# huangzhibo/Hadoop-BAM

Measured on AMD Instinct MI355X. Metric: uncompressed BAM decode GB/s + records/sec per GPU and 8-GPU node, higher is better.
Workload: dtype u8; 1 GPU; C2: synthetic 10M x 150bp paired-end coordinate-sorted BAM; records_per_gpu=10000000, uncompressed_bytes=3401886473, split_bytes_rank0=1410310329, parallelism=FileVirtualSplit per rank x1 (BAMSplitGuesser)

## Files before the change

hadoop-bam_amd/csrc/hbam_abi.cpp:

```cpp
#include "../../include/hbam.h"

#include <hip/hip_runtime.h>

#include <algorithm>
#include <cstdio>
#include <cstdlib>
#include <cstring>
#include <map>
#include <memory>
#include <mutex>
#include <string>
#include <vector>

#include "hbam_deflate_api.h"
#include "hbam_mem.h"
#include "hbam_host.h"
#include "hbam_launch.h"

using hadoop_bam::BAMInputFormat;
using hadoop_bam::BamFile;
using hadoop_bam::BAMRecordReader;
using hadoop_bam::Carry;
using hadoop_bam::FileSplit;
using hadoop_bam::FileVirtualSplit;
// ... 428 lines not shown
  }
  return ctx->cursor.reader_position(i, pos, &ctx->err);
}

int hbam_pipeline_counters(hbam_ctx* ctx, uint64_t out[5]) {
  if (!ctx || !ctx->f) return HBAM_E_STATE;
  hbam::Pipeline& p = ctx->f->pipe();
  out[0] = p.link_fallbacks();
  out[1] = p.link_rewalks();
  out[2] = p.record_fallbacks();
  out[3] = p.inflate_launches();
  out[4] = p.records_after_stop();
  return HBAM_OK;
}

int hbam_inflate_token_count(hbam_ctx* ctx, uint64_t* tokens) {
  *tokens = 0;
  if (!ctx || !ctx->f) return HBAM_E_STATE;
  return ctx->f->pipe().inflate_tokens(tokens) == 0 ? HBAM_OK : HBAM_E_DEVICE;
}

int hbam_inflate_path_counts(hbam_ctx* ctx, uint64_t out[3]) {
  out[0] = out[1] = out[2] = 0;
  if (!ctx || !ctx->f) return HBAM_E_STATE;
  return ctx->f->pipe().inflate_path_counts(out) == 0 ? HBAM_OK : HBAM_E_DEVICE;
}

int hbam_inflate_narrow_counts(hbam_ctx* ctx, uint64_t out[3]) {
  out[0] = out[1] = out[2] = 0;
  if (!ctx || !ctx->f) return HBAM_E_STATE;
// ... 442 lines not shown
  return rc;
}

int hbam_gpu_set_window(hbam_gpu* g, uint64_t window_bytes) {
  g->window = window_bytes ? window_bytes : hadoop_bam::kDefaultWindowBytes;
  if (g->f) g->f->set_window_bytes(g->window);
  return HBAM_OK;
}

int hbam_gpu_set_stringency(hbam_gpu* g, int32_t stringency) {
  if (stringency < HBAM_STRICT || stringency > HBAM_SILENT) {
    g->err = "unknown validation stringency";
    return HBAM_E_ARG;
  }
  g->stringency = stringency;
  return HBAM_OK;
}

int hbam_gpu_run(hbam_gpu* g, int32_t flags, hbam_gpu_stats* st) {
  memset(st, 0, sizeof *st);
  if (!g->f) {
    g->err = "hbam_gpu_run needs a loaded file";
    return HBAM_E_STATE;
  }
  return decode_device(*g->f, g->f->first_record_voff(), ~0ull, flags, st, &g->span, &g->err);
}

int hbam_gpu_index(hbam_gpu* g, int32_t granularity, uint8_t** buf, uint64_t* len, float* ms) {
  *buf = nullptr;
  *len = 0;
// ... 263 lines not shown
```

hadoop-bam_amd/csrc/hbam_kernels.hip:

```cpp
#include <hip/hip_runtime.h>
#include <hipcub/hipcub.hpp>
#include <stddef.h>
#include <stdint.h>

#include "hbam_device.h"
#include "hbam_launch.h"

namespace hbam {

__device__ __forceinline__ uint32_t rfl(uint32_t v) { return __builtin_amdgcn_readfirstlane(v); }
__device__ __forceinline__ uint32_t lane_id() { return __lane_id(); }

__device__ __forceinline__ uint32_t ldu32(const uint8_t* base, uint64_t off) {
  const uint32_t* p = reinterpret_cast<const uint32_t*>(base + (off & ~3ull));
  uint32_t lo = p[0], hi = p[1];
  return __builtin_amdgcn_alignbyte(hi, lo, (uint32_t)(off & 3));
}
__device__ __forceinline__ uint64_t ldu64(const uint8_t* base, uint64_t off) {
  return (uint64_t)ldu32(base, off) | ((uint64_t)ldu32(base, off + 4) << 32);
}

struct __attribute__((aligned(4))) U32x4 { uint32_t x, y, z, w; };
struct __attribute__((aligned(4))) U32x2 { uint32_t x, y; };
struct RecHead {
// ... 88 lines not shown
          s_cand[j] = base + p;
        } else {
          const uint32_t i = atomicAdd(count, 1u);
          if (i < cap) cand[i] = base + p;
        }
      }
    }
    }
  }
  __syncthreads();
  const uint32_t nw = min(s_n, kWgCand);
  if (threadIdx.x == 0) s_base = nw ? atomicAdd(count, nw) : 0u;
  __syncthreads();
  for (uint32_t t = threadIdx.x; t < nw; t += blockDim.x)
    if (s_base + t < cap) cand[s_base + t] = s_cand[t];
}

__global__ void k_bgzf_verify(const uint8_t* __restrict__ file, uint64_t lo, uint64_t hi,
                              const uint64_t* __restrict__ cand, uint32_t n,
                              BlockInfo* __restrict__ blocks, uint32_t* __restrict__ flags, uint32_t partial) {
  uint32_t i = blockIdx.x * blockDim.x + threadIdx.x;
  if (i >= n) return;
  uint64_t c = cand[i];
  if (i == 0 && c != lo) atomicOr(&flags[0], 1u);
  uint32_t total = (ldu32(file, c + 16) & 0xffffu) + 1;
  uint64_t next = c + total;
  uint64_t expect = (i + 1 < n) ? cand[i + 1] : hi;
  if (partial && i + 1 == n && next > hi && total >= 26) {
    flags[2] = 1u;
    return;
// ... 3529 lines not shown
  uint64_t g = (n + bs - 1) / bs;
  if (g < 1) g = 1;
  if (g > cap) g = cap;
  return (unsigned)g;
}

hipError_t launch_bgzf_scan(const uint8_t* file, uint64_t buf_base, uint64_t lo, uint64_t hi, uint64_t* cand,
                            uint32_t cap, uint32_t* count, hipStream_t s) {
  (void)buf_base;
  const uint64_t a = lo & ~15ull;
  const uint64_t nc = (hi - a + 15) / 16;
  hipLaunchKernelGGL(k_bgzf_scan, dim3(grid_for((nc + 3) / 4, 256, HBAM_SCAN_GRID)), dim3(256), 0, s, file + a, hi - a, a, lo,
                     cand, cap, count);
  return hipGetLastError();
}
hipError_t launch_bgzf_verify(const uint8_t* file, uint64_t lo, uint64_t hi, const uint64_t* cand, uint32_t n,
                              BlockInfo* blocks, uint32_t* flags, uint32_t partial, hipStream_t s) {
  if (n == 0) return hipSuccess;
  hipLaunchKernelGGL(k_bgzf_verify, dim3((n + 255) / 256), dim3(256), 0, s, file, lo, hi, cand, n, blocks, flags,
                     partial);
  return hipGetLastError();
}
hipError_t launch_bgzf_walk(const uint8_t* file, uint64_t lo, uint64_t hi, BlockInfo* blocks, uint32_t cap,
                            uint32_t* out, uint32_t partial, hipStream_t s) {
  hipLaunchKernelGGL(k_bgzf_walk, dim3(1), dim3(64), 0, s, file, lo, hi, blocks, cap, out, partial);
  return hipGetLastError();
}
hipError_t launch_block_ustart(BlockInfo* blocks, uint32_t n, uint64_t* tmp_isize, uint64_t* tmp_ustart,
                               void* scan_tmp, size_t* scan_bytes, uint64_t base, hipStream_t s) {
  if (scan_tmp == nullptr) {
// ... 295 lines not shown
```

hadoop-bam_amd/csrc/hbam_launch.h:

```cpp
#pragma once
#include <hip/hip_runtime.h>
#include <stdint.h>

#include "hbam_device.h"

namespace hbam {

struct ChainArgs {
  const uint8_t* u;
  const BlockInfo* blocks;
  uint64_t e_inf, e_true, p0, q_end;
  const uint64_t* dead;
  uint32_t ndead;
  int32_t n_ref;
  uint32_t k0, k1;
  int validate;
  const int32_t* ref_len;
  uint64_t *g, *x, *entry, *summary, *base;
  uint64_t* x2;
  void* scan_tmp;
  size_t scan_bytes;
  uint32_t* cnt;
  int32_t* err;
  unsigned long long* need;
// ... 18 lines not shown
  kStageSerialLink = 1,
  kStageCount = 2,
  kStageEmit = 3,
  kStageWalk = 5,
  kStageLinkCheck = 6,
  kStageRewalk = 7,
  kStageRewalkAll = 8,
};

hipError_t launch_bgzf_scan(const uint8_t* file, uint64_t buf_base, uint64_t lo, uint64_t hi, uint64_t* cand,
                            uint32_t cap, uint32_t* count, hipStream_t s);
hipError_t launch_bgzf_verify(const uint8_t* file, uint64_t lo, uint64_t hi, const uint64_t* cand, uint32_t n,
                              BlockInfo* blocks, uint32_t* flags, uint32_t partial, hipStream_t s);
hipError_t launch_bgzf_walk(const uint8_t* file, uint64_t lo, uint64_t hi, BlockInfo* blocks, uint32_t cap,
                            uint32_t* out, uint32_t partial, hipStream_t s);
hipError_t launch_block_ustart(BlockInfo* blocks, uint32_t n, uint64_t* tmp_isize, uint64_t* tmp_ustart,
                               void* scan_tmp, size_t* scan_bytes, uint64_t base, hipStream_t s);
hipError_t sort_u64(void* tmp, size_t* tmp_bytes, uint64_t* keys_in, uint64_t* keys_out, uint32_t n,
                    hipStream_t s);
hipError_t scan_u32_to_u64(void* tmp, size_t* tmp_bytes, const uint32_t* in, uint64_t* out, uint32_t n,
                           hipStream_t s);
hipError_t launch_huff_tables(const uint8_t* file, const BlockInfo* blocks, uint32_t b0, uint32_t nb,
                              uint8_t* tables, HuffTableInfo* tinfo, const HuffOut* hout, uint32_t round,
                              hipStream_t s);
hipError_t launch_inflate_huff_prebuilt(const uint8_t* file, const BlockInfo* blocks, uint32_t b0, uint32_t nb,
                                        uint64_t chunk_ustart, uint32_t* tokens, HuffOut* hout,
                                        const uint8_t* tables, const HuffTableInfo* tinfo, uint32_t round,
                                        uint32_t defer, uint32_t* flist, uint32_t* pstats, hipStream_t s);
hipError_t huff_lean_occupancy(int* workgroups_per_cu);
hipError_t huff_narrow_occupancy(int* workgroups_per_cu, uint32_t* stage_cap_bytes);
// ... 45 lines not shown
```

hadoop-bam_amd/csrc/hbam_pipeline.cpp:

```cpp
#include "hbam_pipeline.h"

#include <thread>

#include <algorithm>
#include <chrono>
#include <cstdio>
#include <cstdlib>
#include <cstring>

#include "hbam_launch.h"

namespace hbam {

namespace {
constexpr uint32_t kStreamInflateBlocks = 8192;
#ifndef HBAM_INFLATE_CHUNK
#define HBAM_INFLATE_CHUNK 65536
#endif
constexpr uint32_t kInflateChunkBlocks = HBAM_INFLATE_CHUNK;
constexpr int kMaxChainIters = 64;
constexpr int kMaxLinkFix = 4;
constexpr int kMaxFreeStarts = 64;
constexpr uint64_t kOpenEnd = 1ull << 62;
}
// ... 18 lines not shown
      create_stream(&stream_stage_, StreamLevel::kLow) != hipSuccess)
    err_ = "hipStreamCreate failed";
  streams_.s[0] = stream_;
  streams_.s[1] = stream_b_;
  streams_.s[2] = stream_t_;
  streams_.s[3] = stream_copy_;
  streams_.n = 4;
  stage_owner_.s[0] = stream_stage_;
  stage_owner_.s[1] = stream_;
  stage_owner_.n = 2;
  stage_.owner = &stage_owner_;
  own(own_file_, own_spare_, dblocks_, ref_len_, du_, tokens_[0], tokens_[1], hout_, tables_[0], tables_[1],
      tinfo_[0], tinfo_[1], flist_[0], flist_[1], pstats_, g_, x_, x2_, entry_, base_arr_, summary_, dead_, cand_, sorted_, isz_, ust_, cnt_, flags_,
      errv_, need_, rec_pos_, rec_voff_, rcand_, force_, wcnt_, counters_, list_, scan_tmp_, cols_, long_rec_,
      long_n_, wbuf_, woffs_, wbad_, scalars_, fuse_, sort_word_, sort_word2_, sort_slen_, sort_doff_, sort_len_,
      sort_iota_, sort_perm_, sort_tmp_);
  for (auto& e : ev_) (void)hipEventCreate(&e);
  for (auto& e : sync_ev_) (void)hipEventCreateWithFlags(&e, hipEventDisableTiming);
  for (auto& e : tab_ev_) (void)hipEventCreateWithFlags(&e, hipEventDisableTiming);
  for (auto& e : hdone_ev_) (void)hipEventCreateWithFlags(&e, hipEventDisableTiming);
}

Pipeline::~Pipeline() {
  if (stage_thr_.joinable()) stage_thr_.join();
  (void)hipSetDevice(device_);
  (void)streams_.sync();
  (void)stage_owner_.sync();
  streams_.n = 0;
  stage_owner_.n = 0;
  if (rb_buf_) pinned_free(rb_buf_, rb_cap_);
  for (auto& e : ev_) (void)hipEventDestroy(e);
// ... 289 lines not shown
int Pipeline::set_ref_lengths(const std::vector<int32_t>& lens) {
  HIPCHK(ref_len_.reserve(lens.size() + 1));
  if (!lens.empty())
    HIPCHK(hipMemcpyAsync(ref_len_.p, lens.data(), lens.size() * 4, hipMemcpyHostToDevice, stream_));
  HIPCHK(rb_sync(stream_));
  n_ref_len_ = (uint32_t)lens.size();
  return kOk;
}

int Pipeline::locate_range(uint64_t lo, uint64_t hi, bool partial, bool free_start, uint32_t nprev, uint64_t ubase,
                           hipStream_t s, uint32_t* nnew, uint64_t* tail) {
  *nnew = 0;
  *tail = hi;
  const uint8_t* fbase = dfile_ - base_;
  const uint64_t len = hi - lo;
  const uint32_t cap = (uint32_t)std::min<uint64_t>(len / 1024 + 4096, 0x7fffffffu);
  const uint32_t walk_cap = (uint32_t)std::min<uint64_t>(len / 26 + 16, 0x7fffffffu);
  HIPCHK(cand_.reserve(cap));
  HIPCHK(flags_.reserve(5));
  HIPCHK(hipMemsetD32Async(reinterpret_cast<hipDeviceptr_t>(flags_.p), 0, 5, s));
  HIPCHK(hipMemsetD32Async(reinterpret_cast<hipDeviceptr_t>(flags_.p + 2), -1, 1, s));
  HIPCHK(launch_bgzf_scan(fbase, base_, lo, hi, cand_.p, cap, flags_.p, s));
  uint32_t count = 0;
  HIPCHK(rb(&count, flags_.p, 4, s));
  HIPCHK(rb_sync(s));
  bool serial = count > cap || (count == 0 && len > 0);
  if (free_start && count == 0) return kOk;
  uint32_t n = serial ? 0 : count;
  auto queue_table = [&](uint32_t nt) -> int {
    HIPCHK(dblocks_.grow(nprev + nt + 1));
    HIPCHK(isz_.reserve(nt + 1));
    HIPCHK(ust_.reserve(nt + 1));
    size_t sb = 0;
    HIPCHK(launch_block_ustart(dblocks_.p + nprev, nt, isz_.p, ust_.p, nullptr, &sb, ubase, s));
    HIPCHK(scan_tmp_.reserve(sb + 16));
    HIPCHK(launch_block_ustart(dblocks_.p + nprev, nt, isz_.p, ust_.p, scan_tmp_.p, &sb, ubase, s));
    HIPCHK(hblocks_.resize(nprev + nt));
    if (nt) HIPCHK(launch_readback(hblocks_.data() + nprev, dblocks_.p + nprev, nt * sizeof(BlockInfo), s));
    return kOk;
  };
  std::vector<uint64_t> starts;
  if (!serial && n > 0) {
    HIPCHK(dblocks_.grow(nprev + n + 1));
    HIPCHK(sorted_.reserve(n));
    size_t tmp_bytes = 0;
    HIPCHK(sort_u64(nullptr, &tmp_bytes, cand_.p, sorted_.p, n, s));
    HIPCHK(scan_tmp_.reserve(tmp_bytes + 16));
    HIPCHK(sort_u64(scan_tmp_.p, &tmp_bytes, cand_.p, sorted_.p, n, s));
    if (free_start) {
      starts.resize(std::min<uint32_t>(n, kMaxFreeStarts));
      HIPCHK(rb(starts.data(), sorted_.p, starts.size() * 8, s));
      HIPCHK(rb_sync(s));
      lo = starts[0];
    }
    HIPCHK(launch_bgzf_verify(fbase, lo, hi, sorted_.p, n, dblocks_.p + nprev, flags_.p + 1, partial ? 1u : 0u, s));
    uint32_t fl[4];
    uint64_t last = 0;
    HIPCHK(rb(fl, flags_.p + 1, 16, s));
    HIPCHK(rb(&last, sorted_.p + n - 1, 8, s));
    if (int rc = queue_table(n)) return rc;
    HIPCHK(rb_sync(s));
    if (!fl[0] && empty_blocks_ != kEmptyUnknown) empty_blocks_ += fl[3];
    if (fl[0]) serial = true;
    else if (fl[1] != 0xffffffffu) return fail(kErrFormat, "BGZF block with ISIZE > 65536 (unsupported on device)");
    else if (fl[2]) {
      n -= 1;
      *tail = last;
    }
    if (!serial) {
      HIPCHK(hblocks_.resize(nprev + n));
      *nnew = n;
      return kOk;
    }
  }
  if (serial) {
    empty_blocks_ = kEmptyUnknown;
    uint32_t out[4];
// ... 893 lines not shown
```

hadoop-bam_amd/csrc/hbam_pipeline.h:

```cpp
#pragma once
#include "hbam_feed.h"
#include "hbam_mem.h"
#include <hip/hip_runtime.h>
#include <stdint.h>

#include <algorithm>
#include <cstring>
#include <string>
#include <thread>
#include <vector>

#include "hbam_device.h"

namespace hbam {

template <typename T>
struct DevBuf {
  T* p = nullptr;
  size_t n = 0;
  const StreamSet* owner = nullptr;
  DevBuf() = default;
  explicit DevBuf(const StreamSet* o) : owner(o) {}
  DevBuf(const DevBuf&) = delete;
  DevBuf& operator=(const DevBuf&) = delete;
// ... 99 lines not shown
  uint64_t first_voff = 0, last_voff = 0;
  Columns col{};
  const uint8_t* data = nullptr;
};

struct StageTimes {
  float locate = 0, inflate = 0, huff = 0, lz77 = 0, chain = 0, decode = 0;
  float tables = 0;
};

enum class StreamLevel { kNormal, kHigh, kLow };
hipError_t create_stream(hipStream_t* s, StreamLevel level);

enum Stringency : int { kStrict = 0, kLenient = 1, kSilent = 2 };

class Pipeline {
 public:
  explicit Pipeline(int device);
  ~Pipeline();
  Pipeline(const Pipeline&) = delete;
  Pipeline& operator=(const Pipeline&) = delete;

  int device() const { return device_; }
  hipStream_t stream() const { return stream_; }
  const StreamSet& streams() const { return streams_; }
  const std::string& error() const { return err_; }

  hipError_t rb(void* dst, const void* src, size_t bytes, hipStream_t s);
  hipError_t rb_sync(hipStream_t s);
  int copy_from_host(uint8_t* dst, const HostSource& src, uint64_t off, uint64_t len);
// ... 40 lines not shown
  int64_t pos_of_voff(uint64_t voff) const;
  uint64_t voff_of(uint64_t pos) const;
  uint64_t q_end_of(uint64_t vend) const;
  uint32_t block_containing(uint64_t pos) const;

  void set_n_ref(int32_t n) { n_ref_ = n; }
  int32_t n_ref() const { return n_ref_; }
  void set_stringency(int s) { stringency_ = s; }
  int set_ref_lengths(const std::vector<int32_t>& lens);

  uint64_t link_fallbacks() const { return link_fallbacks_; }
  uint64_t link_rewalks() const { return link_rewalks_; }
  uint64_t record_fallbacks() const { return record_fallbacks_; }
  uint64_t records_after_stop() const { return records_after_stop_; }
  uint64_t inflate_launches() const { return inflate_launches_; }
  int inflate_tokens(uint64_t* n);
  int inflate_path_counts(uint64_t out[3]);
  int inflate_narrow_counts(uint64_t out[3]);
  int chain_counters(uint64_t out[4]);
  StageTimes times;
  bool timing = false;

 private:
  int fail(int code, const std::string& msg);
  int locate_range(uint64_t lo, uint64_t hi, bool partial, bool free_start, uint32_t nprev, uint64_t ubase,
                   hipStream_t s, uint32_t* nnew, uint64_t* tail);
  int finish_blocks();
  hipError_t queue_inflate_check(uint32_t b0, uint32_t b1);
  int inflate_verdict(uint32_t b0, uint32_t b1);
  uint32_t infl_first_ = 0xffffffffu;
// ... 38 lines not shown
  uint32_t ndead_ = 0;
  static constexpr uint32_t kEmptyUnknown = 0xffffffffu;
  uint32_t empty_blocks_ = kEmptyUnknown;
  int32_t n_ref_ = 0;
  int stringency_ = kStrict;
  DevBuf<int32_t> ref_len_;
  uint32_t n_ref_len_ = 0;
  uint64_t link_fallbacks_ = 0;
  uint64_t link_rewalks_ = 0;
  uint64_t link_rounds_ = 0;
  uint64_t record_fallbacks_ = 0;
  uint64_t records_after_stop_ = 0;
  uint32_t after_stop_flag_ = 0;
  bool after_stop_pending_ = false;
  uint64_t inflate_launches_ = 0;

  DevBuf<uint8_t> du_;
  std::vector<uint8_t> inflated_;
  DevBuf<uint32_t> tokens_[2];
  DevBuf<HuffOut> hout_;
  DevBuf<uint8_t> tables_[2];
  hipStream_t stream_b_ = nullptr;
  hipStream_t stream_t_ = nullptr;
  hipEvent_t tab_ev_[2];
  hipEvent_t hdone_ev_[2];
  hipEvent_t sync_ev_[4];
  DevBuf<HuffTableInfo> tinfo_[2];
  DevBuf<uint32_t> flist_[2];
  DevBuf<uint32_t> pstats_;

  DevBuf<uint64_t> g_, x_, x2_, entry_, base_arr_, summary_, dead_;
  DevBuf<uint64_t> cand_, sorted_, isz_, ust_;
  DevBuf<uint32_t> cnt_, flags_;
  DevBuf<int32_t> errv_;
  DevBuf<unsigned long long> need_;
  DevBuf<uint64_t> rec_pos_, rec_voff_;
  DevBuf<uint64_t> rcand_, force_;
  DevBuf<uint32_t> wcnt_, counters_;
  DevBuf<uint16_t> list_;
  DevBuf<uint32_t> fuse_;
  DevBuf<uint8_t> scan_tmp_;
  DevBuf<uint8_t> cols_;
  uint64_t cols_cap_ = 0;
  DevBuf<uint64_t> long_rec_;
  DevBuf<uint32_t> long_n_;
  DevBuf<uint8_t> wbuf_;
  DevBuf<uint64_t> woffs_;
  DevBuf<unsigned long long> wbad_;
// ... 20 lines not shown
```

hadoop-bam_amd/hbam/__init__.py:

```python
import ctypes as C
import os
import re

import numpy as np

_PKG = os.path.dirname(os.path.dirname(os.path.abspath(__file__)))
LIB_PATH = os.environ.get("HBAM_LIB") or os.path.join(_PKG, "lib", "libhbam.so")
HEADER_PATH = os.path.join(os.path.dirname(_PKG), "include", "hbam.h")

if not os.path.exists(LIB_PATH):
    raise ImportError(f"{LIB_PATH} is not built: run `make -C hadoop-bam_amd` (libhbam has no CPU fallback)")

_L = C.CDLL(LIB_PATH)

OK, E_FORMAT, E_TRUNC, E_ARG, E_IO, E_DEVICE, E_STATE, E_NOMEM = range(8)
ERROR_NAMES = {1: "SAMFormatException", 2: "FileTruncatedException", 3: "IllegalArgumentException",
               4: "IOException", 5: "DeviceError", 6: "IllegalStateException", 7: "OutOfMemoryError"}

u64, i64, i32, u32, P = C.c_uint64, C.c_int64, C.c_int32, C.c_uint32, C.c_void_p


STRICT, LENIENT, SILENT = 0, 1, 2


# ... 51 lines not shown
_sig("hbam_open_bgzf", C.c_int, [P, u64, C.POINTER(Opts), C.POINTER(P)])
READ_FN = C.CFUNCTYPE(C.c_int64, C.c_void_p, C.c_uint64, C.c_void_p, C.c_uint64)
_sig("hbam_open_reader", C.c_int, [u64, READ_FN, P, C.POINTER(Opts), C.POINTER(P)])
_sig("hbam_close", None, [P])
_sig("hbam_last_error", C.c_char_p, [P])
_sig("hbam_free", None, [P])
_sig("hbam_header", C.c_int, [P, C.POINTER(HeaderInfo)])
_sig("hbam_ref", C.c_int, [P, i32, C.POINTER(C.c_char_p), C.POINTER(i32)])
_sig("hbam_decode_span", C.c_int, [P, u64, u64, u64, C.POINTER(Batch)])
_sig("hbam_decode_span_device", C.c_int, [P, u64, u64, i32, C.POINTER(GpuStats)])
_sig("hbam_reader_position", C.c_int, [P, u64, C.POINTER(u64)])
_sig("hbam_query_intervals", C.c_int, [P, P, u64, P, u64])
_sig("hbam_query_unmapped", C.c_int, [P, u64])
_sig("hbam_query_next", C.c_int, [P, u64, C.POINTER(Batch)])
_sig("hbam_pipeline_counters", C.c_int, [P, C.POINTER(u64)])
_sig("hbam_inflate_token_count", C.c_int, [P, C.POINTER(u64)])
_sig("hbam_inflate_path_counts", C.c_int, [P, C.POINTER(u64)])
_sig("hbam_inflate_narrow_counts", C.c_int, [P, C.POINTER(u64)])
_sig("hbam_chain_counters", C.c_int, [P, C.POINTER(u64)])
_sig("hbam_file_stats", C.c_int, [P, C.POINTER(u64), C.POINTER(u64)])
_sig("hbam_bytes_read", C.c_int, [P, C.POINTER(u64)])
_sig("hbam_prefetch", C.c_int, [P, u64, u64])
_sig("hbam_splitting_index_for_records", C.c_int, [C.POINTER(Opts), P, u64, i32, u64, C.POINTER(P), C.POINTER(u64)])
_sig("hbam_build_splitting_index", C.c_int, [P, i32, C.POINTER(P), C.POINTER(u64)])
_sig("hbam_build_bai", C.c_int, [P, i32, C.POINTER(P), C.POINTER(u64)])
_sig("hbam_splitting_entries", C.c_int, [P, u64, u64, i32, u64, C.POINTER(P), C.POINTER(u64), C.POINTER(u64)])
_sig("hbam_guess_record_starts", C.c_int, [P, P, P, u64, P])
_sig("hbam_guess_record_starts_hdr", C.c_int, [P, i32, P, P, u64, P])
_sig("hbam_guess_bgzf_block_starts", C.c_int, [P, P, P, u64, P])
_sig("hbam_get_splits", C.c_int, [P, P, P, u64, P, u64, P, P, C.POINTER(u64)])
# ... 20 lines not shown
_sig("hbam_gpu_encode_writables", C.c_int, [P, i32, C.POINTER(C.c_float), C.POINTER(u64)])
_sig("hbam_gpu_sort_writables", C.c_int, [P, i32, i32, C.POINTER(C.c_float), C.POINTER(u64)])
_sig("hbam_gpu_fetch_encoded", C.c_int, [P, u64, u64, P])
_sig("hbam_gpu_reload", C.c_int, [P, P, u64, i32, C.POINTER(C.c_float)])
_sig("hbam_gpu_run_streamed", C.c_int, [P, P, u64, u64, C.POINTER(GpuStats)])
_sig("hbam_host_alloc", P, [u64])
_sig("hbam_host_free", None, [P])
_sig("hbam_gpu_d2d_bandwidth", C.c_int, [P, u64, i32, C.POINTER(C.c_float)])
_sig("hbam_bgzf_compress", C.c_int, [C.POINTER(Opts), P, u64, P, u64, i32, i32, i32, C.POINTER(P), C.POINTER(u64)])
_sig("hbam_gpu_bgzf_compress", C.c_int, [P, i32, i32, i32, C.POINTER(C.c_float), C.POINTER(u64)])
_sig("hbam_gpu_fetch_compressed", C.c_int, [P, u64, u64, P])
_sig("hbam_bai_summarize", C.c_int, [P, u64, C.POINTER(BaiSummary)])
_sig("hbam_bai_query", C.c_int, [P, u64, P, u64, C.POINTER(P), C.POINTER(u64)])

BGZF_EOF = 1
SORT_KEY, SORT_COORDINATE = 0, 1
SORT_ORDERS = {"key": SORT_KEY, "coordinate": SORT_COORDINATE}
BAI_METADATA = 1
HTSJDK_BLOCK_SIZE = 65498


def lib():
    return _L


def exported_symbols_from_header(path=HEADER_PATH):
    txt = open(path).read()
    txt = re.sub(r"/\*.*?\*/", "", txt, flags=re.S)
    return sorted(set(re.findall(r"\b(hbam_[a-z0-9_]+)\s*\(", txt)))

# ... 268 lines not shown
        if rc != OK:
            raise self._err(rc)

    def reader_position(self, i):
        v = u64()
        rc = _L.hbam_reader_position(self._h, i, C.byref(v))
        if rc != OK:
            raise self._err(rc)
        return v.value

    def pipeline_counters(self):
        v = (u64 * 5)()
        rc = _L.hbam_pipeline_counters(self._h, v)
        if rc != OK:
            raise self._err(rc)
        return dict(zip(("link_fallbacks", "link_rewalks", "record_fallbacks", "inflate_launches",
                         "records_after_stop"),
                        (int(x) for x in v)))

    def inflate_token_count(self):
        v = u64()
        rc = _L.hbam_inflate_token_count(self._h, C.byref(v))
        if rc != OK:
            raise self._err(rc)
        return int(v.value)

    def inflate_path_counts(self):
        v = (u64 * 3)()
        rc = _L.hbam_inflate_path_counts(self._h, v)
        if rc != OK:
            raise self._err(rc)
        return int(v[0]), int(v[1]), int(v[2])

# ... 309 lines not shown
            self._keep = C.create_string_buffer(bytes(data), len(data))
            ptr, n = self._keep, len(data)
        rc = _L.hbam_gpu_load(self._h, ptr, n)
        if rc != OK:
            raise HbamError(rc, _L.hbam_gpu_error(self._h).decode())
        self._keep = None

    def set_window(self, window_bytes):
        _L.hbam_gpu_set_window(self._h, window_bytes)

    def set_stringency(self, stringency):
        rc = _L.hbam_gpu_set_stringency(self._h, stringency)
        if rc != OK:
            raise HbamError(rc, _L.hbam_gpu_error(self._h).decode())

    def run(self, timing=False, decode=True, digest=False):
        st = GpuStats()
        flags = (1 if timing else 0) | (0 if decode else 2) | (4 if digest else 0)
        rc = _L.hbam_gpu_run(self._h, flags, C.byref(st))
        if rc != OK:
            raise HbamError(rc, _L.hbam_gpu_error(self._h).decode())
        return _stats_dict(st)

    def index(self, granularity=4096):
        p = P()
        n = u64()
        ms = C.c_float()
        rc = _L.hbam_gpu_index(self._h, granularity, C.byref(p), C.byref(n), C.byref(ms))
        if rc != OK:
            raise HbamError(rc, _L.hbam_gpu_error(self._h).decode())
# ... 71 lines not shown
```

include/hbam.h:

```cpp
#ifndef HBAM_H
#define HBAM_H

#include <stdint.h>

#ifdef __cplusplus
extern "C" {
#endif

#define HBAM_OK 0
#define HBAM_E_FORMAT 1
#define HBAM_E_TRUNC 2
#define HBAM_E_ARG 3
#define HBAM_E_IO 4
#define HBAM_E_DEVICE 5
#define HBAM_E_STATE 6
#define HBAM_E_NOMEM 7

#define HBAM_ABI_VERSION 6

#define HBAM_STRICT 0
#define HBAM_LENIENT 1
#define HBAM_SILENT 2

typedef struct hbam_ctx hbam_ctx;
// ... 120 lines not shown
  int32_t status;
  int32_t link_fallbacks;
  int32_t inflate_launches;
  int32_t link_rewalks;
  int32_t windows;
  float ms_tables;
  int32_t record_fallbacks;
  uint64_t key_digest, voff_digest;
} hbam_gpu_stats;
#define HBAM_DIGEST_P 0x100000001b3ull

int hbam_decode_span_device(hbam_ctx *ctx, uint64_t vstart, uint64_t vend, int32_t flags, hbam_gpu_stats *st);

int hbam_pipeline_counters(hbam_ctx *ctx, uint64_t out[5]);

int hbam_inflate_token_count(hbam_ctx *ctx, uint64_t *tokens);

int hbam_inflate_path_counts(hbam_ctx *ctx, uint64_t out[3]);

int hbam_inflate_narrow_counts(hbam_ctx *ctx, uint64_t out[3]);

int hbam_chain_counters(hbam_ctx *ctx, uint64_t out[4]);

int hbam_splitting_entries(hbam_ctx *ctx, uint64_t vstart, uint64_t vend, int32_t granularity, uint64_t ordinal0,
                           uint64_t **entries, uint64_t *n_entries, uint64_t *n_records);

typedef struct hbam_gpu hbam_gpu;

int hbam_gpu_create(int32_t device, hbam_gpu **out);
void hbam_gpu_destroy(hbam_gpu *g);
const char *hbam_gpu_error(hbam_gpu *g);
int hbam_gpu_load(hbam_gpu *g, const void *data, uint64_t len);
int hbam_gpu_set_window(hbam_gpu *g, uint64_t window_bytes);
int hbam_gpu_set_stringency(hbam_gpu *g, int32_t stringency);
int hbam_gpu_run(hbam_gpu *g, int32_t flags, hbam_gpu_stats *stats);
int hbam_gpu_index(hbam_gpu *g, int32_t granularity, uint8_t **buf, uint64_t *len, float *ms);
int hbam_gpu_run_streamed(hbam_gpu *g, const void *data, uint64_t len, uint64_t piece_bytes, hbam_gpu_stats *st);
void *hbam_host_alloc(uint64_t bytes);
void hbam_host_free(void *p);
int hbam_gpu_reload(hbam_gpu *g, const void *data, uint64_t len, int32_t pinned, float *ms);
int hbam_gpu_d2d_bandwidth(hbam_gpu *g, uint64_t bytes, int32_t iters, float *gbps);
int hbam_gpu_encode_writables(hbam_gpu *g, int32_t iters, float *ms_per_iter, uint64_t *bytes);
int hbam_gpu_fetch_encoded(hbam_gpu *g, uint64_t pos, uint64_t len, uint8_t *dst);
int hbam_gpu_sort_writables(hbam_gpu *g, int32_t order, int32_t iters, float ms[3], uint64_t *bytes);
int hbam_gpu_bgzf_compress(hbam_gpu *g, int32_t level, int32_t flags, int32_t iters, float *ms_per_iter,
                           uint64_t *out_len);
int hbam_gpu_fetch_compressed(hbam_gpu *g, uint64_t pos, uint64_t len, uint8_t *dst);
int hbam_gpu_fetch(hbam_gpu *g, int64_t *keys, uint64_t *voffs, uint64_t cap);
int32_t hbam_device_count(void);
// ... 6 lines not shown
```

Baseline: 229.1 GB/s.

## Locate BGZF blocks by per-segment anchor walks instead of full scan and sort

Adds a segmented BGZF block locator. One wave per 512 KiB segment finds the first verified header (two chained headers), walks the block chain serially, and links segments with a block scan. A final emit kernel writes the sorted block offsets. This replaces the byte-wise candidate scan and radix sort when the chain links cleanly, and falls back to the old scan otherwise. The cost is an extra host readback and sync, plus serial per-lane walking within each segment.

```diff
diff --git a/hadoop-bam_amd/csrc/hbam_abi.cpp b/hadoop-bam_amd/csrc/hbam_abi.cpp
--- a/hadoop-bam_amd/csrc/hbam_abi.cpp
+++ b/hadoop-bam_amd/csrc/hbam_abi.cpp
@@ -466,6 +466,32 @@
   return HBAM_OK;
 }
 
+namespace {
+void set_locate(BamFile& f, uint64_t seg_bytes, uint32_t cap_limit) {
+  hbam::Pipeline& p = f.pipe();
+  if (seg_bytes == HBAM_LOCATE_SEG_DEFAULT) {
+    seg_bytes = hbam::kLocateSegBytes;
+    if (const char* e = getenv("HBAM_LOCATE_SEG")) seg_bytes = strtoull(e, nullptr, 0);
+  }
+  p.set_locate(seg_bytes, cap_limit);
+  f.invalidate_window();
+}
+}
+
+int hbam_locate_counters(hbam_ctx* ctx, uint64_t out[2]) {
+  out[0] = out[1] = 0;
+  if (!ctx || !ctx->f) return HBAM_E_STATE;
+  out[0] = ctx->f->pipe().locate_anchored();
+  out[1] = ctx->f->pipe().locate_declined();
+  return HBAM_OK;
+}
+
+int hbam_set_locate(hbam_ctx* ctx, uint64_t seg_bytes, uint32_t cap_limit) {
+  if (!ctx || !ctx->f) return HBAM_E_STATE;
+  set_locate(*ctx->f, seg_bytes, cap_limit);
+  return HBAM_OK;
+}
+
 int hbam_inflate_token_count(hbam_ctx* ctx, uint64_t* tokens) {
   *tokens = 0;
   if (!ctx || !ctx->f) return HBAM_E_STATE;
@@ -938,6 +964,23 @@
     return HBAM_E_ARG;
   }
   g->stringency = stringency;
+  return HBAM_OK;
+}
+
+int hbam_gpu_set_locate(hbam_gpu* g, uint64_t seg_bytes, uint32_t cap_limit) {
+  if (!g->f) {
+    g->err = "hbam_gpu_set_locate needs a loaded file";
+    return HBAM_E_STATE;
+  }
+  set_locate(*g->f, seg_bytes, cap_limit);
+  return HBAM_OK;
+}
+
+int hbam_gpu_locate_counters(hbam_gpu* g, uint64_t out[2]) {
+  out[0] = out[1] = 0;
+  if (!g->f) return HBAM_E_STATE;
+  out[0] = g->f->pipe().locate_anchored();
+  out[1] = g->f->pipe().locate_declined();
   return HBAM_OK;
 }
 
diff --git a/hadoop-bam_amd/csrc/hbam_kernels.hip b/hadoop-bam_amd/csrc/hbam_kernels.hip
--- a/hadoop-bam_amd/csrc/hbam_kernels.hip
+++ b/hadoop-bam_amd/csrc/hbam_kernels.hip
@@ -126,6 +126,165 @@
   __syncthreads();
   for (uint32_t t = threadIdx.x; t < nw; t += blockDim.x)
     if (s_base + t < cap) cand[s_base + t] = s_cand[t];
+}
+
+constexpr uint64_t kNoAnchor = ~0ull;
+#ifndef HBAM_ANCHOR_U
+#define HBAM_ANCHOR_U 4
+#endif
+
+__device__ __forceinline__ bool bgzf_header_at(const uint8_t* __restrict__ file, uint64_t p, uint32_t* total) {
+  const uint32_t w0 = ldu32(file, p);
+  const uint32_t xlen = ldu32(file, p + 10) & 0xffffu;
+  const uint32_t sub = ldu32(file, p + 12);
+  *total = (ldu32(file, p + 16) & 0xffffu) + 1;
+  return w0 == 0x04088b1fu && xlen == 6 && sub == 0x00024342u && *total >= 26;
+}
+
+__device__ __forceinline__ uint64_t wave_min_u64(uint64_t v) {
+#pragma unroll
+  for (int o = 32; o; o >>= 1) {
+    const uint32_t l2 = (uint32_t)__shfl_xor((int)(uint32_t)v, o, 64);
+    const uint32_t h2 = (uint32_t)__shfl_xor((int)(uint32_t)(v >> 32), o, 64);
+    const uint64_t v2 = ((uint64_t)h2 << 32) | l2;
+    v = v2 < v ? v2 : v;
+  }
+  return v;
+}
+
+__global__ __launch_bounds__(256) void k_bgzf_anchor_walk(const uint8_t* __restrict__ file, uint64_t lo, uint64_t hi,
+                                                          uint64_t seg, uint32_t nseg, uint32_t partial,
+                                                          uint64_t* __restrict__ anchor, uint64_t* __restrict__ exitp,
+                                                          uint32_t* __restrict__ cnt, uint32_t* __restrict__ res) {
+  const uint32_t j = blockIdx.x * (blockDim.x / 64) + threadIdx.x / 64;
+  if (j >= nseg) return;
+  const uint32_t lane = lane_id();
+  const uint64_t s0 = lo + (uint64_t)j * seg;
+  const uint64_t end = s0 + seg < hi ? s0 + seg : hi;
+  uint64_t a = j == 0 ? lo : kNoAnchor;
+  if (j != 0) {
+    constexpr int kU = HBAM_ANCHOR_U;
+    const uint4* chunks = reinterpret_cast<const uint4*>(file);
+    const uint64_t cend = (end + 15) / 16;
+    auto fetch = [&](uint64_t c0, uint4* vv, uint32_t& tail) {
+#pragma unroll
+      for (int u = 0; u < kU; ++u) {
+        const uint64_t c = c0 + 64 * u + lane;
+        vv[u] = c < cend ? chunks[c] : make_uint4(0, 0, 0, 0);
+      }
+      const uint64_t clast = c0 + 64 * (kU - 1) + 63;
+      tail = lane == 63 && clast < cend ? *reinterpret_cast<const uint32_t*>(file + 16 * clast + 16) : 0u;
+    };
+    uint4 nv[kU];
+    uint32_t ntail = 0;
+    const uint64_t cfirst = s0 / 16;
+    fetch(cfirst, nv, ntail);
+    for (uint64_t c0 = cfirst; c0 < cend && a == kNoAnchor; c0 += 64 * kU) {
+      uint4 vv[kU];
+#pragma unroll
+      for (int u = 0; u < kU; ++u) vv[u] = nv[u];
+      const uint32_t tail = ntail;
+      if (c0 + 64 * kU < cend) fetch(c0 + 64 * kU, nv, ntail);
+      uint64_t best = kNoAnchor;
+#pragma unroll
+      for (int u = 0; u < kU; ++u) {
+        const uint64_t c = c0 + 64 * u + lane;
+        const uint4 v = vv[u];
+        uint32_t nx = (uint32_t)__shfl_down((int)v.x, 1, 64);
+        const uint32_t next0 = u + 1 < kU ? (uint32_t)__shfl((int)vv[u + 1 < kU ? u + 1 : u].x, 0, 64) : 0u;
+        if (lane == 63) nx = u + 1 < kU ? next0 : tail;
+        const uint32_t w[5] = {v.x, v.y, v.z, v.w, nx};
+#pragma unroll
+        for (int k = 0; k < 4; ++k) {
+          const uint32_t x = w[k] ^ 0x1f1f1f1fu;
+          uint32_t hz = (x - 0x01010101u) & ~x & 0x80808080u;
+          while (hz) {
+            const uint32_t byte = (uint32_t)__builtin_ctz(hz) >> 3;
+            hz &= hz - 1;
+            if (__builtin_amdgcn_alignbyte(w[k + 1], w[k], byte) != 0x04088b1fu) continue;
+            const uint64_t p = 16 * c + 4 * k + byte;
+            if (p < s0 || p >= end || p + 18 > hi || p >= best) continue;
+            uint32_t total, t2;
+            if (!bgzf_header_at(file, p, &total)) continue;
+            const uint64_t q = p + total;
+            if (q < hi && (q + 18 > hi || !bgzf_header_at(file, q, &t2))) continue;
+            best = p;
+          }
+        }
+      }
+      if (__any(best != kNoAnchor)) a = wave_min_u64(best);
+    }
+  }
+  if (lane != 0) return;
+  uint64_t p = a;
+  uint32_t n = 0;
+  if (a != kNoAnchor) {
+    while (p < end) {
+      uint32_t total;
+      if (p + 18 > hi || !bgzf_header_at(file, p, &total)) {
+        atomicOr(&res[0], 1u);
+        break;
+      }
+      ++n;
+      p += total;
+      if (p > hi) {
+        if (!partial) atomicOr(&res[0], 1u);
+        break;
+      }
+    }
+  }
+  anchor[j] = a;
+  exitp[j] = a != kNoAnchor ? p : kNoAnchor;
+  cnt[j] = n;
+}
+
+constexpr int kLinkThreads = 1024;
+struct LastExitOp {
+  __device__ __forceinline__ uint64_t operator()(uint64_t x, uint64_t y) const { return y != kNoAnchor ? y : x; }
+};
+__global__ __launch_bounds__(kLinkThreads) void k_bgzf_link(const uint64_t* __restrict__ anchor,
+                                                            const uint64_t* __restrict__ exitp,
+                                                            const uint32_t* __restrict__ cnt, uint32_t nseg,
+                                                            uint64_t hi, uint32_t* __restrict__ offs,
+                                                            uint32_t* __restrict__ res) {
+  using ScanSum = hipcub::BlockScan<uint64_t, kLinkThreads>;
+  __shared__ typename ScanSum::TempStorage tmp;
+  const uint32_t per = (nseg + kLinkThreads - 1) / kLinkThreads;
+  const uint32_t j0 = min(threadIdx.x * per, nseg), j1 = min(j0 + per, nseg);
+  uint64_t sum = 0, last = kNoAnchor;
+  for (uint32_t j = j0; j < j1; ++j) {
+    sum += cnt[j];
+    if (anchor[j] != kNoAnchor) last = exitp[j];
+  }
+  uint64_t before = 0, prev = kNoAnchor, total = 0;
+  ScanSum(tmp).ExclusiveSum(sum, before, total);
+  __syncthreads();
+  ScanSum(tmp).ExclusiveScan(last, prev, kNoAnchor, LastExitOp());
+  bool bad = false;
+  for (uint32_t j = j0; j < j1; ++j) {
+    offs[j] = before < 0xffffffffull ? (uint32_t)before : 0xffffffffu;
+    before += cnt[j];
+    const uint64_t a = anchor[j];
+    if (a == kNoAnchor) continue;
+    if (prev != kNoAnchor && prev != a) bad = true;
+    prev = exitp[j];
+  }
+  if (threadIdx.x == kLinkThreads - 1 && (prev == kNoAnchor || prev < hi)) bad = true;
+  if (bad) atomicOr(&res[0], 1u);
+  if (threadIdx.x == 0) res[1] = total < 0xffffffffull ? (uint32_t)total : 0xffffffffu;
+}
+
+__global__ void k_bgzf_seg_emit(const uint8_t* __restrict__ file, const uint64_t* __restrict__ anchor,
+                                const uint32_t* __restrict__ cnt, const uint32_t* __restrict__ offs, uint32_t nseg,
+                                uint32_t cap, uint64_t* __restrict__ out) {
+  const uint32_t j = blockIdx.x * blockDim.x + threadIdx.x;
+  if (j >= nseg) return;
+  uint64_t p = anchor[j];
+  const uint32_t n = cnt[j], o = offs[j];
+  for (uint32_t i = 0; i < n && o + i < cap; ++i) {
+    out[o + i] = p;
+    p += (ldu32(file, p + 16) & 0xffffu) + 1;
+  }
 }
 
 __global__ void k_bgzf_verify(const uint8_t* __restrict__ file, uint64_t lo, uint64_t hi,
@@ -3685,6 +3844,19 @@
                      cand, cap, count);
   return hipGetLastError();
 }
+hipError_t launch_bgzf_anchor_walk(const uint8_t* file, uint64_t lo, uint64_t hi, uint64_t seg, uint32_t nseg,
+                                   uint32_t partial, uint64_t* anchor, uint64_t* exitp, uint32_t* cnt, uint32_t* offs,
+                                   uint32_t* res, hipStream_t s) {
+  hipLaunchKernelGGL(k_bgzf_anchor_walk, dim3((nseg + 3) / 4), dim3(256), 0, s, file, lo, hi, seg, nseg, partial,
+                     anchor, exitp, cnt, res);
+  hipLaunchKernelGGL(k_bgzf_link, dim3(1), dim3(kLinkThreads), 0, s, anchor, exitp, cnt, nseg, hi, offs, res);
+  return hipGetLastError();
+}
+hipError_t launch_bgzf_seg_emit(const uint8_t* file, const uint64_t* anchor, const uint32_t* cnt,
+                                const uint32_t* offs, uint32_t nseg, uint32_t n, uint64_t* out, hipStream_t s) {
+  hipLaunchKernelGGL(k_bgzf_seg_emit, dim3((nseg + 63) / 64), dim3(64), 0, s, file, anchor, cnt, offs, nseg, n, out);
+  return hipGetLastError();
+}
 hipError_t launch_bgzf_verify(const uint8_t* file, uint64_t lo, uint64_t hi, const uint64_t* cand, uint32_t n,
                               BlockInfo* blocks, uint32_t* flags, uint32_t partial, hipStream_t s) {
   if (n == 0) return hipSuccess;
diff --git a/hadoop-bam_amd/csrc/hbam_launch.h b/hadoop-bam_amd/csrc/hbam_launch.h
--- a/hadoop-bam_amd/csrc/hbam_launch.h
+++ b/hadoop-bam_amd/csrc/hbam_launch.h
@@ -56,6 +56,11 @@
                               BlockInfo* blocks, uint32_t* flags, uint32_t partial, hipStream_t s);
 hipError_t launch_bgzf_walk(const uint8_t* file, uint64_t lo, uint64_t hi, BlockInfo* blocks, uint32_t cap,
                             uint32_t* out, uint32_t partial, hipStream_t s);
+hipError_t launch_bgzf_anchor_walk(const uint8_t* file, uint64_t lo, uint64_t hi, uint64_t seg, uint32_t nseg,
+                                   uint32_t partial, uint64_t* anchor, uint64_t* exitp, uint32_t* cnt, uint32_t* offs,
+                                   uint32_t* res, hipStream_t s);
+hipError_t launch_bgzf_seg_emit(const uint8_t* file, const uint64_t* anchor, const uint32_t* cnt,
+                                const uint32_t* offs, uint32_t nseg, uint32_t n, uint64_t* out, hipStream_t s);
 hipError_t launch_block_ustart(BlockInfo* blocks, uint32_t n, uint64_t* tmp_isize, uint64_t* tmp_ustart,
                                void* scan_tmp, size_t* scan_bytes, uint64_t base, hipStream_t s);
 hipError_t sort_u64(void* tmp, size_t* tmp_bytes, uint64_t* keys_in, uint64_t* keys_out, uint32_t n,
diff --git a/hadoop-bam_amd/csrc/hbam_pipeline.cpp b/hadoop-bam_amd/csrc/hbam_pipeline.cpp
--- a/hadoop-bam_amd/csrc/hbam_pipeline.cpp
+++ b/hadoop-bam_amd/csrc/hbam_pipeline.cpp
@@ -56,7 +56,8 @@
       tinfo_[0], tinfo_[1], flist_[0], flist_[1], pstats_, g_, x_, x2_, entry_, base_arr_, summary_, dead_, cand_, sorted_, isz_, ust_, cnt_, flags_,
       errv_, need_, rec_pos_, rec_voff_, rcand_, force_, wcnt_, counters_, list_, scan_tmp_, cols_, long_rec_,
       long_n_, wbuf_, woffs_, wbad_, scalars_, fuse_, sort_word_, sort_word2_, sort_slen_, sort_doff_, sort_len_,
-      sort_iota_, sort_perm_, sort_tmp_);
+      sort_iota_, sort_perm_, sort_tmp_, seg_anchor_, seg_exit_, seg_cnt_, seg_off_);
+  if (const char* e = getenv("HBAM_LOCATE_SEG")) locate_seg_ = strtoull(e, nullptr, 0);
   for (auto& e : ev_) (void)hipEventCreate(&e);
   for (auto& e : sync_ev_) (void)hipEventCreateWithFlags(&e, hipEventDisableTiming);
   for (auto& e : tab_ev_) (void)hipEventCreateWithFlags(&e, hipEventDisableTiming);
@@ -376,16 +377,40 @@
   *tail = hi;
   const uint8_t* fbase = dfile_ - base_;
   const uint64_t len = hi - lo;
-  const uint32_t cap = (uint32_t)std::min<uint64_t>(len / 1024 + 4096, 0x7fffffffu);
+  uint32_t cap = (uint32_t)std::min<uint64_t>(len / 1024 + 4096, 0x7fffffffu);
+  if (locate_cap_limit_) cap = std::min(cap, locate_cap_limit_);
   const uint32_t walk_cap = (uint32_t)std::min<uint64_t>(len / 26 + 16, 0x7fffffffu);
   HIPCHK(cand_.reserve(cap));
-  HIPCHK(flags_.reserve(5));
-  HIPCHK(hipMemsetD32Async(reinterpret_cast<hipDeviceptr_t>(flags_.p), 0, 5, s));
+  HIPCHK(flags_.reserve(8));
+  HIPCHK(hipMemsetD32Async(reinterpret_cast<hipDeviceptr_t>(flags_.p), 0, 7, s));
   HIPCHK(hipMemsetD32Async(reinterpret_cast<hipDeviceptr_t>(flags_.p + 2), -1, 1, s));
-  HIPCHK(launch_bgzf_scan(fbase, base_, lo, hi, cand_.p, cap, flags_.p, s));
   uint32_t count = 0;
-  HIPCHK(rb(&count, flags_.p, 4, s));
-  HIPCHK(rb_sync(s));
+  bool anchored = false;
+  if (!free_start && locate_seg_ && len > 0 && (len + locate_seg_ - 1) / locate_seg_ <= 0x7fffffffu) {
+    const uint32_t nseg = (uint32_t)((len + locate_seg_ - 1) / locate_seg_);
+    HIPCHK(seg_anchor_.reserve(nseg));
+    HIPCHK(seg_exit_.reserve(nseg));
+    HIPCHK(seg_cnt_.reserve(nseg));
+    HIPCHK(seg_off_.reserve(nseg));
+    HIPCHK(launch_bgzf_anchor_walk(fbase, lo, hi, locate_seg_, nseg, partial ? 1u : 0u, seg_anchor_.p, seg_exit_.p,
+                                   seg_cnt_.p, seg_off_.p, flags_.p + 5, s));
+    uint32_t res[2] = {1, 0};
+    HIPCHK(rb(res, flags_.p + 5, 8, s));
+    HIPCHK(rb_sync(s));
+    if (!res[0] && res[1] > 0 && res[1] <= cap) {
+      count = res[1];
+      HIPCHK(sorted_.reserve(count));
+      HIPCHK(launch_bgzf_seg_emit(fbase, seg_anchor_.p, seg_cnt_.p, seg_off_.p, nseg, count, sorted_.p, s));
+      anchored = true;
+    } else {
+      ++locate_declined_;
+    }
+  }
+  if (!anchored) {
+    HIPCHK(launch_bgzf_scan(fbase, base_, lo, hi, cand_.p, cap, flags_.p, s));
+    HIPCHK(rb(&count, flags_.p, 4, s));
+    HIPCHK(rb_sync(s));
+  }
   bool serial = count > cap || (count == 0 && len > 0);
   if (free_start && count == 0) return kOk;
   uint32_t n = serial ? 0 : count;
@@ -404,11 +429,13 @@
   std::vector<uint64_t> starts;
   if (!serial && n > 0) {
     HIPCHK(dblocks_.grow(nprev + n + 1));
-    HIPCHK(sorted_.reserve(n));
-    size_t tmp_bytes = 0;
-    HIPCHK(sort_u64(nullptr, &tmp_bytes, cand_.p, sorted_.p, n, s));
-    HIPCHK(scan_tmp_.reserve(tmp_bytes + 16));
-    HIPCHK(sort_u64(scan_tmp_.p, &tmp_bytes, cand_.p, sorted_.p, n, s));
+    if (!anchored) {
+      HIPCHK(sorted_.reserve(n));
+      size_t tmp_bytes = 0;
+      HIPCHK(sort_u64(nullptr, &tmp_bytes, cand_.p, sorted_.p, n, s));
+      HIPCHK(scan_tmp_.reserve(tmp_bytes + 16));
+      HIPCHK(sort_u64(scan_tmp_.p, &tmp_bytes, cand_.p, sorted_.p, n, s));
+    }
     if (free_start) {
       starts.resize(std::min<uint32_t>(n, kMaxFreeStarts));
       HIPCHK(rb(starts.data(), sorted_.p, starts.size() * 8, s));
@@ -423,6 +450,7 @@
     if (int rc = queue_table(n)) return rc;
     HIPCHK(rb_sync(s));
     if (!fl[0] && empty_blocks_ != kEmptyUnknown) empty_blocks_ += fl[3];
+    if (anchored) ++(fl[0] ? locate_declined_ : locate_anchored_);
     if (fl[0]) serial = true;
     else if (fl[1] != 0xffffffffu) return fail(kErrFormat, "BGZF block with ISIZE > 65536 (unsupported on device)");
     else if (fl[2]) {
diff --git a/hadoop-bam_amd/csrc/hbam_pipeline.h b/hadoop-bam_amd/csrc/hbam_pipeline.h
--- a/hadoop-bam_amd/csrc/hbam_pipeline.h
+++ b/hadoop-bam_amd/csrc/hbam_pipeline.h
@@ -137,6 +137,11 @@
 
 enum Stringency : int { kStrict = 0, kLenient = 1, kSilent = 2 };
 
+#ifndef HBAM_LOCATE_SEG_BYTES
+#define HBAM_LOCATE_SEG_BYTES (512u << 10)
+#endif
+constexpr uint64_t kLocateSegBytes = HBAM_LOCATE_SEG_BYTES;
+
 class Pipeline {
  public:
   explicit Pipeline(int device);
@@ -207,6 +212,13 @@
   uint64_t record_fallbacks() const { return record_fallbacks_; }
   uint64_t records_after_stop() const { return records_after_stop_; }
   uint64_t inflate_launches() const { return inflate_launches_; }
+  uint64_t locate_anchored() const { return locate_anchored_; }
+  uint64_t locate_declined() const { return locate_declined_; }
+  void set_locate(uint64_t seg_bytes, uint32_t cap_limit) {
+    locate_seg_ = seg_bytes;
+    locate_cap_limit_ = cap_limit;
+  }
+  uint64_t locate_seg() const { return locate_seg_; }
   int inflate_tokens(uint64_t* n);
   int inflate_path_counts(uint64_t out[3]);
   int inflate_narrow_counts(uint64_t out[3]);
@@ -275,6 +287,9 @@
   uint32_t after_stop_flag_ = 0;
   bool after_stop_pending_ = false;
   uint64_t inflate_launches_ = 0;
+  uint64_t locate_anchored_ = 0, locate_declined_ = 0;
+  uint64_t locate_seg_ = kLocateSegBytes;
+  uint32_t locate_cap_limit_ = 0;
 
   DevBuf<uint8_t> du_;
   std::vector<uint8_t> inflated_;
@@ -293,6 +308,8 @@
   DevBuf<uint64_t> g_, x_, x2_, entry_, base_arr_, summary_, dead_;
   DevBuf<uint64_t> cand_, sorted_, isz_, ust_;
   DevBuf<uint32_t> cnt_, flags_;
+  DevBuf<uint64_t> seg_anchor_, seg_exit_;
+  DevBuf<uint32_t> seg_cnt_, seg_off_;
   DevBuf<int32_t> errv_;
   DevBuf<unsigned long long> need_;
   DevBuf<uint64_t> rec_pos_, rec_voff_;
diff --git a/hadoop-bam_amd/hbam/__init__.py b/hadoop-bam_amd/hbam/__init__.py
--- a/hadoop-bam_amd/hbam/__init__.py
+++ b/hadoop-bam_amd/hbam/__init__.py
@@ -89,6 +89,10 @@
 _sig("hbam_query_unmapped", C.c_int, [P, u64])
 _sig("hbam_query_next", C.c_int, [P, u64, C.POINTER(Batch)])
 _sig("hbam_pipeline_counters", C.c_int, [P, C.POINTER(u64)])
+_sig("hbam_locate_counters", C.c_int, [P, C.POINTER(u64)])
+_sig("hbam_set_locate", C.c_int, [P, u64, u32])
+_sig("hbam_gpu_set_locate", C.c_int, [P, u64, u32])
+_sig("hbam_gpu_locate_counters", C.c_int, [P, C.POINTER(u64)])
 _sig("hbam_inflate_token_count", C.c_int, [P, C.POINTER(u64)])
 _sig("hbam_inflate_path_counts", C.c_int, [P, C.POINTER(u64)])
 _sig("hbam_inflate_narrow_counts", C.c_int, [P, C.POINTER(u64)])
@@ -139,6 +143,7 @@
 _sig("hbam_bai_query", C.c_int, [P, u64, P, u64, C.POINTER(P), C.POINTER(u64)])
 
 BGZF_EOF = 1
+LOCATE_SEG_DEFAULT = (1 << 64) - 1
 SORT_KEY, SORT_COORDINATE = 0, 1
 SORT_ORDERS = {"key": SORT_KEY, "coordinate": SORT_COORDINATE}
 BAI_METADATA = 1
@@ -437,9 +442,18 @@
         rc = _L.hbam_pipeline_counters(self._h, v)
         if rc != OK:
             raise self._err(rc)
+        w = (u64 * 2)()
+        rc = _L.hbam_locate_counters(self._h, w)
+        if rc != OK:
+            raise self._err(rc)
         return dict(zip(("link_fallbacks", "link_rewalks", "record_fallbacks", "inflate_launches",
-                         "records_after_stop"),
-                        (int(x) for x in v)))
+                         "records_after_stop", "locate_anchored", "locate_declined"),
+                        (int(x) for x in list(v) + list(w))))
+
+    def set_locate(self, seg_bytes=LOCATE_SEG_DEFAULT, cap_limit=0):
+        rc = _L.hbam_set_locate(self._h, seg_bytes, cap_limit)
+        if rc != OK:
+            raise self._err(rc)
 
     def inflate_token_count(self):
         v = u64()
@@ -779,6 +793,18 @@
         if rc != OK:
             raise HbamError(rc, _L.hbam_gpu_error(self._h).decode())
 
+    def set_locate(self, seg_bytes=LOCATE_SEG_DEFAULT, cap_limit=0):
+        rc = _L.hbam_gpu_set_locate(self._h, seg_bytes, cap_limit)
+        if rc != OK:
+            raise HbamError(rc, _L.hbam_gpu_error(self._h).decode())
+
+    def locate_counters(self):
+        w = (u64 * 2)()
+        rc = _L.hbam_gpu_locate_counters(self._h, w)
+        if rc != OK:
+            raise HbamError(rc, _L.hbam_gpu_error(self._h).decode())
+        return int(w[0]), int(w[1])
+
     def run(self, timing=False, decode=True, digest=False):
         st = GpuStats()
         flags = (1 if timing else 0) | (0 if decode else 2) | (4 if digest else 0)
diff --git a/include/hbam.h b/include/hbam.h
--- a/include/hbam.h
+++ b/include/hbam.h
@@ -158,6 +158,10 @@
 
 int hbam_pipeline_counters(hbam_ctx *ctx, uint64_t out[5]);
 
+int hbam_locate_counters(hbam_ctx *ctx, uint64_t out[2]);
+#define HBAM_LOCATE_SEG_DEFAULT UINT64_MAX
+int hbam_set_locate(hbam_ctx *ctx, uint64_t seg_bytes, uint32_t cap_limit);
+
 int hbam_inflate_token_count(hbam_ctx *ctx, uint64_t *tokens);
 
 int hbam_inflate_path_counts(hbam_ctx *ctx, uint64_t out[3]);
@@ -177,6 +181,8 @@
 int hbam_gpu_load(hbam_gpu *g, const void *data, uint64_t len);
 int hbam_gpu_set_window(hbam_gpu *g, uint64_t window_bytes);
 int hbam_gpu_set_stringency(hbam_gpu *g, int32_t stringency);
+int hbam_gpu_set_locate(hbam_gpu *g, uint64_t seg_bytes, uint32_t cap_limit);
+int hbam_gpu_locate_counters(hbam_gpu *g, uint64_t out[2]);
 int hbam_gpu_run(hbam_gpu *g, int32_t flags, hbam_gpu_stats *stats);
 int hbam_gpu_index(hbam_gpu *g, int32_t granularity, uint8_t **buf, uint64_t *len, float *ms);
 int hbam_gpu_run_streamed(hbam_gpu *g, const void *data, uint64_t len, uint64_t piece_bytes, hbam_gpu_stats *st);
```

Measured after the change: 233.3 GB/s (median of 6 runs). +1.8%, better.
